# ConwayBeyond/Funscript-Flow

Hardware: AMD Instinct MI355X
Metric: 1080p frame-pairs/sec (higher is better)
Workload: dtype f32

## Files before the change

### funscript_flow_amd/csrc/ffl_api.hip

```cpp
#include "../../include/ffl.h"
#include "ffl_kernels.h"

#include <math.h>
#include <stdarg.h>
#include <stdio.h>
#include <string.h>

#include <algorithm>
#include <condition_variable>
#include <mutex>
#include <string>
#include <thread>
#include <vector>

#define FFL_EV_RING 16
#define FFL_RAW_RING 4

template <class H, class Arg, hipError_t (*Free)(Arg)>
struct Owned {
    H h = H();
    Owned() = default;
    explicit Owned(H take) : h(take) {}
    Owned(Owned &&o) noexcept : h(o.release()) {}
    Owned &operator=(Owned &&o) noexcept { std::swap(h, o.h); return *this; }
// ... 1120 lines not shown
    } pl[3];
    const size_t cw = (size_t)sw / 2 * es, ch = (size_t)sh / 2;
    const size_t wrow = (size_t)yw.w * es, x0 = (size_t)yw.x0 * es;
    pl[0] = {(size_t)yw.y0 * stride_bytes + x0, 0, stride_bytes, wrow, yw.h};
    int np = 3;
    if (nv12) {
        pl[1] = {(size_t)(sh + yw.y0 / 2) * stride_bytes + x0, ybytes, stride_bytes, wrow, yw.h / 2};
        np = 2;
    } else {
        const size_t u0 = (size_t)sh * sw * es + (size_t)(yw.y0 / 2) * cw + x0 / 2;
        pl[1] = {u0, ybytes, (ptrdiff_t)cw, wrow / 2, yw.h / 2};
        pl[2] = {u0 + ch * cw, ybytes + ybytes / 4, (ptrdiff_t)cw, wrow / 2, yw.h / 2};
    }
    const size_t span = (size_t)stride_bytes * (sh + sh / 2 - 1) + (size_t)sw * es;
    auto direct = [&](int i) {
        bool ok = in_host_buf(c, frames[i], span);
        for (int k = 0; ok && k < np; k++) ok = ((uintptr_t)(frames[i] + pl[k].src) | (size_t)pl[k].pitch | pl[k].row) % 4 == 0;
        return ok;
    };
    auto stage = [&](int i, uint8_t *h, int threads) {
        const uint8_t *src[2] = {frames[i] + pl[0].src, nullptr};
        c->pool.copy(h, src, 1, pl[0].pitch, pl[0].row, pl[0].rows, threads);
        src[0] = frames[i] + pl[1].src;
        if (!nv12) src[1] = frames[i] + pl[2].src;
        c->pool.copy(h + pl[1].dst, src, nv12 ? 1 : 2, pl[1].pitch, pl[1].row, pl[1].rows, threads);
    };
    auto send_direct = [&](int i, uint8_t *d) -> int {
        for (int k = 0; k < np; k++)
            HIPCHK(c, hipMemcpy2DAsync(d + pl[k].dst, pl[k].row, frames[i] + pl[k].src, (size_t)pl[k].pitch, pl[k].row,
                                       (size_t)pl[k].rows, hipMemcpyHostToDevice, c->s_copy));
        return FFL_OK;
    };
    auto desc = [&](const uint8_t *d) {
        FrameDesc s = {};
        s.p0 = d;
        s.p1 = d + ybytes;
        s.p2 = nv12 ? s.p1 + es : s.p1 + ybytes / 4;
        s.pitch0 = wrow;
        s.pitch1 = s.pitch2 = nv12 ? wrow : wrow / 2;
        s.c_step = (nv12 ? 2 : 1) * es;
        s.wx = yw.x0;
        s.wy = yw.y0;
        return s;
    };
    return upload_staged(c, lk, first, n, fbytes, fp, direct, stage, send_direct, desc);
}

int ffl_upload_frames_yuv(ffl_ctx *c, int first, int n, const uint8_t *const *frames, int sw, int sh, ptrdiff_t stride_bytes,
                          int layout, int rw, int rh, int crop_x, int crop_y) {
    return upload_yuv(c, "ffl_upload_frames_yuv", first, n, frames, sw, sh, stride_bytes, layout, 1, 8, 0, rw, rh, crop_x, crop_y,
                      nullptr);
}

int ffl_upload_frames_yuv_src(ffl_ctx *c, int first, int n, const uint8_t *const *frames, int sw, int sh, ptrdiff_t stride_bytes,
                              int layout, int rw, int rh, int crop_x, int crop_y, const ffl_source_info *si) {
    return upload_yuv(c, "ffl_upload_frames_yuv", first, n, frames, sw, sh, stride_bytes, layout, 1, 8, 0, rw, rh, crop_x, crop_y, si);
}

int ffl_upload_frames_yuv16(ffl_ctx *c, int first, int n, const uint16_t *const *frames, int sw, int sh, ptrdiff_t stride_bytes,
                            int layout, int depth, int msb_aligned, int rw, int rh, int crop_x, int crop_y) {
    return upload_yuv(c, "ffl_upload_frames_yuv16", first, n, (const uint8_t *const *)frames, sw, sh, stride_bytes, layout, 2,
                      depth, msb_aligned != 0, rw, rh, crop_x, crop_y, nullptr);
}

int ffl_upload_frames_yuv16_src(ffl_ctx *c, int first, int n, const uint16_t *const *frames, int sw, int sh, ptrdiff_t stride_bytes,
                                int layout, int depth, int msb_aligned, int rw, int rh, int crop_x, int crop_y,
                                const ffl_source_info *si) {
    return upload_yuv(c, "ffl_upload_frames_yuv16", first, n, (const uint8_t *const *)frames, sw, sh, stride_bytes, layout, 2,
                      depth, msb_aligned != 0, rw, rh, crop_x, crop_y, si);
}

int ffl_upload_frame(ffl_ctx *c, int fslot, const uint8_t *data, int width, int height, int channels,
                     ptrdiff_t stride_bytes) {
    return ffl_upload_frames(c, fslot, 1, &data, width, height, channels, stride_bytes);
}

int ffl_download_frame(ffl_ctx *c, int fslot, uint8_t *dst) {
    if (!c) return FFL_ERR_INVALID;
    CtxLock lk(c->mu);
    if (!dst || fslot < 0 || fslot >= c->n_fslots)
        return set_err(c, FFL_ERR_INVALID, "ffl_download_frame: bad frame slot %d", fslot);
    if (!c->frame_valid[fslot]) return set_err(c, FFL_ERR_STATE, "ffl_download_frame: frame slot %d was never uploaded", fslot);
    HIPCHK(c, hipSetDevice(c->device));
    HIPCHK(c, hipMemcpyAsync(dst, c->d_gray + (size_t)fslot * c->N, c->N, hipMemcpyDeviceToHost, c->s_copy));
    HIPCHK(c, hipStreamSynchronize(c->s_copy));
    return FFL_OK;
}

struct DebugCapture {
    int level, iter;
    float *I0, *I1, *R0, *R1, *M, *flow;
};

static int enqueue_batch(ffl_ctx *c, ffl_ctx::Lane &L, const BatchTab &T, int n, int nU, int pov_mode, const DebugCapture *cap) {
    hipStream_t st = L.st;
    const size_t N = c->N;
    const UTab *ut = &L.d_tab->ut;
    const PairTab *pt = &L.d_tab->pt;
    auto pyr_level = [&](int k, hipStream_t s) { ffl_launch_pyr_level(c->d_gray, N, ut, nU, L.pyr[c->geo.levels - k], s); };
    auto expand_level = [&](int k, hipStream_t s) {
        {
            ProfScope ps(c, FFL_K_PYRAMID, s);
            pyr_level(k, s);
        }
        {
            ProfScope ps(c, FFL_K_POLYEXP, s);
            ffl_launch_polyexp(L.poly[c->geo.levels - k], nU, c->pc, s);
        }
    };
    const int mode = cap ? 0 : c->opt.run_ahead;
    if (mode) {
        for (int k = 0; k < (mode == 2 ? 4 : 1); k++)
            if (!L.st_aux[k]) HIPCHK(c, hipStreamCreateWithFlags(L.st_aux[k].put(), hipStreamNonBlocking));
        HIPCHK(c, hipEventRecord(L.ev_fork, st));
        for (int k = c->geo.levels; k >= 0; k--) {
            hipStream_t sa = L.st_aux[mode == 2 ? k : 0];
            if (mode == 2 || k == c->geo.levels) HIPCHK(c, hipStreamWaitEvent(sa, L.ev_fork, 0));
            expand_level(k, sa);
            HIPCHK(c, hipEventRecord(L.ev_R[k], sa));
        }
        if (mode == 2)
            for (int k = c->geo.levels; k >= 0; k--) HIPCHK(c, hipStreamWaitEvent(st, L.ev_R[k], 0));
    }
    const bool run_ahead = mode == 1;
    bool expanded = mode != 0;
    if (mode == 0 && c->opt.merge_expand) {
        const PyrJob *l0 = &L.pyr[L.n_jobs - 1];
        const bool fuse_l0 = c->opt.fuse_l0_blur && ffl_polyexp_from_gray_ok(*l0);
        const int skip_l0 = fuse_l0 && !cap;
        {
            ProfScope ps(c, FFL_K_PYRAMID, st);
            if (!ffl_launch_pyr_multi(c->d_gray, N, ut, nU, L.pyr, L.n_jobs - skip_l0, c->opt, st))
                for (int k = c->geo.levels; k >= skip_l0; k--) pyr_level(k, st);
        }
        {
            ProfScope ps(c, FFL_K_POLYEXP, st);
            ffl_launch_polyexp_multi(L.poly, L.n_jobs, nU, c->pc, c->d_gray, N, ut, fuse_l0 ? l0 : nullptr, st);
        }
        expanded = true;
    }

    int pw = 0, ph = 0;
    for (int k = c->geo.levels; k >= 0; k--) {
        const LevelGeom &g = c->geo.lv[k];
        const int lw = g.lw, lh = g.lh;
        const size_t plane = (size_t)lw * lh;
        const size_t I_stride = plane, R_stride = 5 * plane, M_stride = 5 * plane;
        float *Rk = L.d_R + c->lay.r_off[k];
        if (pw == 0 && cap)
            for (int i = 0; i < n; i++) HIPCHK(c, hipMemsetAsync(T.pt.flow[k][i], 0, sizeof(float) * 2 * plane, st));
        if (run_ahead) HIPCHK(c, hipStreamWaitEvent(st, L.ev_R[k], 0));
        else if (!expanded) expand_level(k, st);
        int mi = 0;
        const bool fuse_first = c->opt.fuse_first > 0 && !cap && (long)((lw + 63) / 64) * ((lh + 15) / 16) * n >= c->opt.fuse_first;
        if (!fuse_first) {
            ProfScope ps(c, FFL_K_UPDATE_MATRICES, st);
            ffl_launch_update_matrices(Rk, R_stride, plane, pt, k, n, L.d_M[mi], M_stride, lw, lh, pw, ph, pw == 0, cap != nullptr, c->opt, st);
        }
        bool captured = false;
        auto capture = [&]() -> int {
            HIPCHK(c, hipStreamSynchronize(st));
            if (cap->I0) HIPCHK(c, hipMemcpy(cap->I0, L.d_I + c->lay.i_off[k] + (size_t)T.pt.u0[0] * I_stride, sizeof(float) * plane, hipMemcpyDeviceToHost));
            if (cap->I1) HIPCHK(c, hipMemcpy(cap->I1, L.d_I + c->lay.i_off[k] + (size_t)T.pt.u1[0] * I_stride, sizeof(float) * plane, hipMemcpyDeviceToHost));
            if (cap->R0) HIPCHK(c, hipMemcpy(cap->R0, Rk + (size_t)T.pt.u0[0] * R_stride, sizeof(float) * 5 * plane, hipMemcpyDeviceToHost));
            if (cap->R1) HIPCHK(c, hipMemcpy(cap->R1, Rk + (size_t)T.pt.u1[0] * R_stride, sizeof(float) * 5 * plane, hipMemcpyDeviceToHost));
            if (cap->M) HIPCHK(c, hipMemcpy(cap->M, L.d_M[mi], sizeof(float) * 5 * plane, hipMemcpyDeviceToHost));
            if (cap->flow) HIPCHK(c, hipMemcpy(cap->flow, T.pt.flow[k][0], sizeof(float) * 2 * plane, hipMemcpyDeviceToHost));
            captured = true;
            return FFL_OK;
        };
        for (int it = 0; it < 3; it++) {
            if (cap && cap->level == k && cap->iter == it) {
                int rc = capture();
                if (rc) return rc;
            }
            const int update = it < 2;
            {
                ProfScope ps(c, FFL_K_BLUR_SOLVE, st, it > 0 && !cap);
                if (it == 0 && fuse_first)
                    ffl_launch_blur_solve_first(L.d_M[mi ^ 1], M_stride, Rk, R_stride, plane, pt, k, n, lw, lh, pw, ph, c->opt, st);
                else
                    ffl_launch_blur_solve(L.d_M[mi], L.d_M[mi ^ 1], M_stride, Rk, R_stride, plane, pt, k, n, lw, lh,
                                          update, cap != nullptr, c->opt, st);
            }
            if (update) mi ^= 1;
        }
        if (cap && cap->level == k && !captured) {
            int rc = capture();
            if (rc) return rc;
        }
        pw = lw;
        ph = lh;
    }
    {
        ProfScope ps(c, FFL_K_PASS1, st);
        ffl_launch_pass1(pt, n, c->w, c->h, pov_mode, L.d_pkey, L.d_psum, st);
    }
    return FFL_OK;
}

static int batch_graph(ffl_ctx *c, ffl_ctx::Lane &L, const BatchTab &T, int n, int nU, int pov_mode,
                       ffl_ctx::Lane::GraphEntry **ge) {
    *ge = nullptr;
    for (auto &g : L.graphs)
        if (g.n == n && g.nU == nU && g.pov == pov_mode && g.epoch == c->opt_epoch) *ge = &g;
    if (*ge || c->graph_bad_epoch == c->opt_epoch) return FFL_OK;
    hipStream_t st = L.st;
    ffl_ctx::Lane::GraphEntry g = {n, nU, pov_mode, c->opt_epoch, Graph(), GraphExec()};
    hipError_t fail = hipStreamBeginCapture(st, hipStreamCaptureModeThreadLocal);
    if (fail == hipSuccess) {
        const int rc = enqueue_batch(c, L, T, n, nU, pov_mode, nullptr);
        fail = hipStreamEndCapture(st, g.graph.put());
        if (fail == hipSuccess && (rc != FFL_OK || !g.graph)) fail = hipErrorStreamCaptureInvalidated;
        if (fail == hipSuccess) fail = hipGraphInstantiate(g.exec.put(), g.graph, nullptr, nullptr, 0);
    }
    if (fail != hipSuccess) {
        g.exec.reset();
        g.graph.reset();
        (void)hipGetLastError();
        c->graph_bad_epoch = c->opt_epoch;
        c->graph_failed++;
        if (!c->graph_fail_reported) {
            c->graph_fail_reported = true;
            fprintf(stderr, "libffl_hip: hipGraph capture of a %d-pair batch failed (%s); this context launches its batches "
                            "one kernel at a time until its options change (results are unaffected)\n", n, hipGetErrorString(fail));
        }
        return FFL_OK;
    }
    if (L.graphs.size() >= 16) {
        HIPCHK(c, hipStreamSynchronize(st));
        L.graphs.erase(L.graphs.begin());
    }
    L.graphs.push_back(std::move(g));
    *ge = &L.graphs.back();
    c->graph_captured++;
    return FFL_OK;
}

static int fbg_work(ffl_ctx *c, ffl_ctx::Lane &L, const FbgPlan &p, int nU, FbgWork *wk);

static int queue_batch(ffl_ctx *c, ffl_ctx::Lane &L, BatchTab &T, int *nU_out, int n, const int *f0, const int *f1,
                       const int *slots, int pov_mode, const DebugCapture *cap, const DisKParams *dis,
                       const FbgPlan *fbg) {
    hipStream_t st = L.st;
    const size_t N = c->N;
    int nU = 0;
    auto uidx = [&](int fs) {
        int &u = c->u_of_fslot[fs];
        if (u < 0) {
            T.ut.fslot[nU] = fs;
            u = nU++;
        }
        return u;
    };
    for (int i = 0; i < n; i++) {
        T.pt.u0[i] = uidx(f0[i]);
        T.pt.u1[i] = uidx(f1[i]);
        T.pt.res[i] = c->d_res + slots[i];
    }
    for (int k = c->geo.levels; k >= 0; k--) {
        const size_t plane = (size_t)c->geo.lv[k].lw * c->geo.lv[k].lh;
        float *buf = ((c->geo.levels - k) & 1) ? L.d_flowB : L.d_flowA;
        for (int i = 0; i < n; i++)
            T.pt.flow[k][i] = (k == 0) ? c->d_flow + (size_t)slots[i] * 2 * N : buf + (size_t)i * 2 * plane;
    }
    for (int k = c->geo.levels + 1; k < FFL_MAX_LEVELS; k++)
        for (int i = 0; i < n; i++) T.pt.flow[k][i] = nullptr;
    for (int i = 0; i < nU; i++) c->u_of_fslot[T.ut.fslot[i]] = -1;
    *nU_out = nU;
    WaitOnce wait(st);
    for (int i = 0; i < nU; i++) HIPCHK(c, wait(c->ev_uploaded[T.ut.fslot[i]].get()));
    for (int i = 0; i < n; i++) HIPCHK(c, wait(c->ev_slot_done[slots[i]].get()));
    HIPCHK(c, hipMemcpyAsync(L.d_tab, &T, sizeof(BatchTab), hipMemcpyHostToDevice, st));

    if (fbg || dis) {
        if (fbg) {
            FbgWork wk;
            if (int rc = fbg_work(c, L, *fbg, nU, &wk)) return rc;
            ffl_launch_fb_general(&L.d_tab->ut, &L.d_tab->pt, n, nU, c->d_gray, N, c->w, c->h, *fbg, wk, st);
        } else {
            ffl_launch_dis(&L.d_tab->ut, &L.d_tab->pt, n, c->d_gray, N, L.d_M[0], *dis, st);
        }
        ProfScope ps(c, FFL_K_PASS1, st);
        ffl_launch_pass1(&L.d_tab->pt, n, c->w, c->h, pov_mode, L.d_pkey, L.d_psum, st);
    } else if (c->opt.use_graph && !cap && c->prof_mask == 0 && c->opt.run_ahead == 0) {
        ffl_ctx::Lane::GraphEntry *ge;
        if (int rc = batch_graph(c, L, T, n, nU, pov_mode, &ge)) return rc;
        if (ge) {
            HIPCHK(c, hipGraphLaunch(ge->exec, st));
            c->graph_replayed++;
        } else if (int rc = enqueue_batch(c, L, T, n, nU, pov_mode, nullptr)) {
            return rc;
        }
    } else if (int rc = enqueue_batch(c, L, T, n, nU, pov_mode, cap)) {
        return rc;
    }
    HIPCHK(c, hipGetLastError());
    return FFL_OK;
}

static int run_batch(ffl_ctx *c, int li, int n, const int *f0, const int *f1, const int *slots, int pov_mode,
                     const DebugCapture *cap, const DisKParams *dis = nullptr, const FbgPlan *fbg = nullptr) {
    ffl_ctx::Lane &L = c->lanes[li];
    HIPCHK(c, L.ring.settle_next());
    BatchTab &T = L.h_tab[L.ring.next % FFL_EV_RING];
    int nU = 0;
// ... 959 lines not shown
```

### funscript_flow_amd/csrc/ffl_kernels.h

```cpp
#pragma once
#include <hip/hip_runtime.h>
#include <limits.h>
#include <stdint.h>

#define FFL_MAXB 256
#define FFL_MAXU (2 * FFL_MAXB)
#define FFL_MAX_LEVELS 4
#define FFL_POLY_N 5
#define FFL_WIN 15
#define FFL_WIN_R 7

struct PolyConsts {
    float g[FFL_POLY_N + 1], xg[FFL_POLY_N + 1], xxg[FFL_POLY_N + 1];
    double gd[FFL_POLY_N + 1], xxgd[FFL_POLY_N + 1];
    double ig11, ig03, ig33, ig55;
};

struct GaussKernel {
    float k[32];
    int ksize;
};

struct UTab {
    int fslot[FFL_MAXU];
};

struct PairTab {
    int u0[FFL_MAXB], u1[FFL_MAXB];
    float *flow[FFL_MAX_LEVELS][FFL_MAXB];
    struct Pass1Result *res[FFL_MAXB];
};

struct BatchTab {
    UTab ut;
    PairTab pt;
};

struct Pass1Result {
    int x, y;
    float div_val;
    float pad;
    double mag_sum;
};

enum { FFL_FRONT_GENERIC = 0, FFL_FRONT_AREA2 = 1, FFL_FRONT_IDENTITY = 2 };
enum { FFL_SRC_GRAY = 0, FFL_SRC_BGR = 1, FFL_SRC_YUV = 2, FFL_SRC_YUV16 = 3, FFL_SRC_ANY = -1 };
struct FrameDesc {
    const uint8_t *p0, *p1, *p2;
    long long pitch0, pitch1, pitch2;
    long long ps, cs;
    int c_step;
    int wx, wy;
    int fslot;
};
struct FrontParams {
    int kind, rgb;
    int sw, sh;
    int cx, cy, ow, oh;
    double scale_x, scale_y;
    int mode;
    int shift16, round16;
    int src;
    int ax, bx, cx0, ay, by, cy0;
    int full;
};
struct ExportTab {
    int slot[FFL_MAXB];
};

enum { FFL_IMP_F32 = 0, FFL_IMP_F16 = 1, FFL_IMP_BF16 = 2 };
enum { FFL_IMP_ANY = 0,
       FFL_IMP_NHWC = 1,
       FFL_IMP_NCHW = 2 };
struct ImportArgs {
    const char *base;
    long long item, pitch, ps, cs;
    float *flow;
    Pass1Result *res;
};

#define FFL_MAX_JOBS 4
enum { FFL_PYR_NONE = -1, FFL_PYR_F1 = 0, FFL_PYR_F2, FFL_PYR_H4, FFL_PYR_H9, FFL_PYR_V4, FFL_PYR_V9, FFL_PYR_H1 };
struct PyrJob {
    int kind, w, h, lw, lh;
    unsigned gx, gy, first, count;
    double sx, sy;
    float *tmp, *I;
    size_t tmp_stride, I_stride;
    GaussKernel gk;
};
struct PyrJobs {
    PyrJob j[FFL_MAX_JOBS];
    int n;
};
struct PolyJob {
    const float *I;
    float *R;
    size_t I_stride, R_stride, plane;
    int w, h;
    unsigned gx, gy, first, count;
    int from_gray;
    float gk0, gk1;
};
struct PolyJobs {
    PolyJob j[FFL_MAX_JOBS];
    int n;
};

struct FflOptions {
    int lanes = 2;
    int run_ahead = 0;
    int fuse_first = 10000;
    int merge_expand = 1;
    int use_graph = 1;
    int copy_threads = 4;
    int blur_rows = 0;
    int blur_min_wgs = 3500;
    int tile_order = 0;
    int pyr_coarse = 1;
    int fuse_l0_blur = 1;
    int fb_general = 0;
    int import_fused = 1;
};
struct FflOptionRow {
    const char *name;
    int FflOptions::*member;
    int lo, hi;
    bool flag;
};
inline constexpr FflOptionRow kFflOptionRows[] = {
    {"lanes", &FflOptions::lanes, 1, 4, false},
    {"run_ahead", &FflOptions::run_ahead, 0, 2, false},
    {"fuse_first", &FflOptions::fuse_first, 0, INT_MAX, false},
    {"merge_expand", &FflOptions::merge_expand, INT_MIN, INT_MAX, true},
    {"graph", &FflOptions::use_graph, INT_MIN, INT_MAX, true},
    {"copy_threads", &FflOptions::copy_threads, 1, 16, false},
    {"blur_rows", &FflOptions::blur_rows, 0, 64, false},
    {"blur_min_wgs", &FflOptions::blur_min_wgs, 1, INT_MAX, false},
    {"tile_order", &FflOptions::tile_order, 0, 1, false},
    {"pyr_coarse", &FflOptions::pyr_coarse, INT_MIN, INT_MAX, true},
    {"fuse_l0_blur", &FflOptions::fuse_l0_blur, INT_MIN, INT_MAX, true},
    {"fb_general", &FflOptions::fb_general, 0, 1, false},
    {"import_fused", &FflOptions::import_fused, 0, 1, false},
};

bool ffl_launch_pyr_multi(const uint8_t *gray_base, size_t gray_stride, const UTab *ut, int nU, const PyrJob *levels, int n,
                          const FflOptions &opt, hipStream_t st);
bool ffl_polyexp_from_gray_ok(const PyrJob &l0);
void ffl_launch_polyexp_multi(const PolyJob *levels, int n, int nU, PolyConsts pc, const uint8_t *gray_base, size_t gray_stride,
                              const UTab *ut, const PyrJob *l0, hipStream_t st);
void ffl_launch_frontend(const FrameDesc &d, uint8_t *gray, const FrontParams &p, hipStream_t st);
void ffl_launch_frontend_dev(const FrameDesc *tab, int n, uint8_t *gray_base, size_t N, const FrontParams &p, hipStream_t st);
void ffl_launch_export_flows(const float *flow, const ExportTab &tab, int n, size_t N, char *dst, long long item_stride,
                             int layout, hipStream_t st);
void ffl_launch_import_pass1(const ImportArgs &a, const ExportTab &tab, int n, int dtype, int mode, int w, int h, int pov_mode,
                             int fused, PairTab *pt, unsigned long long *pkey, double *psum, hipStream_t st);
void ffl_launch_gray(const uint8_t *bgr, uint8_t *gray, int n_pixels, hipStream_t st);
size_t ffl_pyr_tmp_floats(int w, int h, int lw);
bool ffl_pyr_level_ok(int w, int h, int lw, int lh, int ksize);
void ffl_launch_pyr_level(const uint8_t *gray_base, size_t gray_stride, const UTab *ut, int nU, const PyrJob &level,
                          hipStream_t st);
void ffl_launch_polyexp(const PolyJob &level, int nU, PolyConsts pc, hipStream_t st);
void ffl_launch_update_matrices(const float *R, size_t R_stride, size_t plane, const PairTab *pt, int level, int nB, float *M,
                                size_t M_stride, int lw, int lh, int pw, int ph, int zero_flow, int store_flow,
                                const FflOptions &opt, hipStream_t st);
void ffl_launch_blur_solve(const float *Min, float *Mout, size_t M_stride, const float *R, size_t R_stride,
                           size_t plane, const PairTab *pt, int level, int nB, int lw, int lh, int update, int store_flow,
                           const FflOptions &opt, hipStream_t st);


void ffl_launch_blur_solve_first(float *Mout, size_t M_stride, const float *R, size_t R_stride, size_t plane,
                                 const PairTab *pt, int level, int nB, int lw, int lh, int pw, int ph, const FflOptions &opt,
                                 hipStream_t st);

#define DIS_MAX_PATCHES 4096
#define DIS_MAX_SCALES 12
struct DisKParams {
    int w, h, finest, coarsest, stride, gd_iters, vr_iters, mean_norm, spatial_prop, stripes;
    float alpha, gamma, delta;
    size_t pair_floats;
    size_t pyr_floats;
    size_t pyr_off[DIS_MAX_SCALES];
    float *dbg;
    int dbg_scale, dbg_stage;
};
void ffl_launch_dis(const UTab *ut, const PairTab *pt, int nB, const uint8_t *gray, size_t gray_stride, float *scratch,
                    const DisKParams &p, hipStream_t st);

int ffl_pass1_blocks(int w, int h);
void ffl_launch_pass1(const PairTab *pt, int nB, int w, int h, int pov_mode, unsigned long long *pkey, double *psum,
                      hipStream_t st);

#define FFL_WINDOW_MAX_RADIUS 32
struct WindowSeq {
    int slot[FFL_MAXB + 2 * FFL_WINDOW_MAX_RADIUS];
};
struct WindowItem {
    const float *flow;
    double cx, cy;
    int cut, pad;
};
struct Pass2Record {
    double dot, cx, cy;
    float mean_mag, div_val;
    int x, y, cut, pad;
};
void ffl_launch_radial(const WindowItem *tab, int n, int w, int h, int pov_mode, const double *wytab, double *psum,
                       Pass2Record *out, hipStream_t st);
void ffl_launch_window_plan(const WindowSeq &seq, int n_seq, int first, int n, int radius, float cut_threshold,
                            const Pass1Result *res, const float *flow, int w, int h, WindowItem *tab, Pass2Record *out,
                            hipStream_t st);

__device__ __forceinline__ int ffl_clampi(int v, int lo, int hi) { return v < lo ? lo : (v > hi ? hi : v); }

__device__ __forceinline__ int ffl_reflect101(int p, int n) {
    if (n == 1) return 0;
    while (p < 0 || p >= n) p = p < 0 ? -p : 2 * (n - 1) - p;
    return p;
}

__device__ __forceinline__ void ffl_resize_coord(int d, int src, double scale, int &i0, int &i1, float &f) {
    float fx = (float)((d + 0.5) * scale - 0.5);
    int sx = (int)floorf(fx);
    fx -= sx;
    if (sx < 0) { sx = 0; fx = 0.f; }
    if (sx >= src - 1) { sx = src - 1; fx = 0.f; }
    i0 = sx;
    i1 = sx + 1 < src ? sx + 1 : src - 1;
    f = fx;
}

static inline unsigned ffl_xcd_blocks(unsigned count) { return ((count + 7) / 8) * 8; }
__device__ __forceinline__ bool ffl_xcd_tile(unsigned l, unsigned count, unsigned &t) {
    const unsigned chunk = (count + 7) >> 3;
    t = (l & 7u) * chunk + (l >> 3);
    return (l >> 3) < chunk && t < count;
}

#ifndef FFL_PANEL_W
#define FFL_PANEL_W 4
#endif
static inline unsigned ffl_tile_grid(int tiles_x, int tiles_y, int nB) {
    const int T = tiles_x * tiles_y;
    return (unsigned)(((T + 7) / 8) * 8 * nB);
}
__device__ __forceinline__ bool ffl_tile_coord(int tiles_x, int tiles_y, int nB, int order, int &b, int &tile_x,
                                               int &tile_y) {
    const int T = tiles_x * tiles_y, chunk = (T + 7) >> 3;
    int t;
    if (order == 0) {
        b = blockIdx.x / (chunk * 8);
        const int l = blockIdx.x - b * (chunk * 8);
        t = (l & 7) * chunk + (l >> 3);
    } else {
        const int pos = blockIdx.x >> 3, tt = pos / nB;
        b = pos - tt * nB;
        t = (blockIdx.x & 7) * chunk + tt;
    }
    if (t >= T) return false;
    const int per_panel = FFL_PANEL_W * tiles_y;
    const int panel = t / per_panel, within = t - panel * per_panel;
    const int pw = min(FFL_PANEL_W, tiles_x - panel * FFL_PANEL_W);
    tile_y = within / pw;
    tile_x = panel * FFL_PANEL_W + (within - tile_y * pw);
    return true;
}

#define FFL_GLOBAL __attribute__((address_space(1)))
typedef float ffl_v2f __attribute__((ext_vector_type(2), aligned(4)));
typedef float ffl_v4f __attribute__((ext_vector_type(4), aligned(4)));
__device__ __forceinline__ float2 ffl_gload2(const void *base, size_t byte_off) {
    const ffl_v2f v = *(const FFL_GLOBAL ffl_v2f *)((const char *)base + byte_off);
    return make_float2(v.x, v.y);
}
__device__ __forceinline__ float4 ffl_gload4(const void *base, size_t byte_off) {
    const ffl_v4f v = *(const FFL_GLOBAL ffl_v4f *)((const char *)base + byte_off);
    return make_float4(v.x, v.y, v.z, v.w);
}

struct __attribute__((packed, aligned(4))) ffl_f2u { float x, y; };
struct __attribute__((packed, aligned(4))) ffl_f4u { float x, y, z, w; };

template <typename T>
__device__ __forceinline__ const T *ffl_at(const float *base, unsigned idx) {
    return reinterpret_cast<const T *>(reinterpret_cast<const char *>(base) + idx * 4u);
}
template <typename T>
__device__ __forceinline__ T *ffl_at(float *base, unsigned idx) {
    return reinterpret_cast<T *>(reinterpret_cast<char *>(base) + idx * 4u);
}

__device__ __forceinline__ ffl_f2u ffl_ld_corner(const float *plane_base, unsigned idx) {
    ffl_f2u v;
    v.x = *ffl_at<float>(plane_base, idx);
    v.y = *ffl_at<float>(plane_base, idx + 1u);
    return v;
}

struct UmLoc {
    int x1, y1;
    float a00, a01, a10, a11;
    bool inside;
};
__device__ __forceinline__ UmLoc ffl_um_locate(int w, int h, int x, int y, float dx, float dy) {
    UmLoc L;
    float fx = x + dx, fy = y + dy;
    L.x1 = (int)floorf(fx);
    L.y1 = (int)floorf(fy);
    fx -= L.x1;
    fy -= L.y1;
    L.inside = (unsigned)L.x1 < (unsigned)(w - 1) && (unsigned)L.y1 < (unsigned)(h - 1);
    L.a00 = (1.f - fx) * (1.f - fy);
    L.a01 = fx * (1.f - fy);
    L.a10 = (1.f - fx) * fy;
    L.a11 = fx * fy;
    return L;
}

__device__ __forceinline__ void ffl_um_finish(const float (&r0)[5], const float (&b)[5], bool inside, int w, int h, int x,
                                              int y, float dx, float dy, float (&out)[5]) {
#define FFL_BORDER(i) ((i) < 2 ? 0.14f : 0.4472f)
    float r2 = inside ? b[0] : 0.f;
    float r3 = inside ? b[1] : 0.f;
    float r4 = inside ? (r0[2] + b[2]) * 0.5f : r0[2];
    float r5 = inside ? (r0[3] + b[3]) * 0.5f : r0[3];
    float r6 = inside ? (r0[4] + b[4]) * 0.25f : r0[4] * 0.5f;
    r2 = (r0[0] - r2) * 0.5f;
// ... 53 lines not shown
```

### funscript_flow_amd/csrc/kernels_farneback.hip

```cpp
#include "ffl_kernels.h"

__global__ __launch_bounds__(256) void k_gray(const uint8_t *__restrict__ bgr, uint8_t *__restrict__ gray, int n) {
    int i4 = (blockIdx.x * 256 + threadIdx.x) * 4;
    if (i4 + 3 < n) {
        const uint32_t *p = reinterpret_cast<const uint32_t *>(bgr + (size_t)i4 * 3);
        uint32_t a = p[0], b = p[1], c = p[2];
        uint32_t px[12] = {a & 255, (a >> 8) & 255, (a >> 16) & 255, a >> 24, b & 255, (b >> 8) & 255,
                           (b >> 16) & 255, b >> 24, c & 255, (c >> 8) & 255, (c >> 16) & 255, c >> 24};
        uint32_t o = 0;
#pragma unroll
        for (int j = 0; j < 4; j++) {
            uint32_t g = (px[j * 3] * 3735u + px[j * 3 + 1] * 19235u + px[j * 3 + 2] * 9798u + 16384u) >> 15;
            o |= g << (8 * j);
        }
        *reinterpret_cast<uint32_t *>(gray + i4) = o;
    } else {
        for (int i = i4; i < n; i++) {
            uint32_t b = bgr[(size_t)i * 3], g = bgr[(size_t)i * 3 + 1], r = bgr[(size_t)i * 3 + 2];
            gray[i] = (uint8_t)((b * 3735u + g * 19235u + r * 9798u + 16384u) >> 15);
        }
    }
}

void ffl_launch_gray(const uint8_t *bgr, uint8_t *gray, int n_pixels, hipStream_t st) {
// ... 1094 lines not shown
                const unsigned lane_byte = ((unsigned)((c0 + vcc) * plane) + (unsigned)vgx) * 4u;
                if (FIRST) {
#pragma unroll
                    for (int j = 0; j < NCARRY; j++) v[j] = carry[g][j];
#pragma unroll
                    for (int j = 0; j < TH; j++)
                        v[NCARRY + j] = g == 0 ? sM012[(vcc * TH + j) * UP + vtx] : sM34[c0 - GC + vcc][j][vtx];
                } else {
                    if (rb == 0) {
#pragma unroll
                        for (int j = 0; j < NCARRY; j++) {
                            const unsigned gy = (unsigned)min(max(y0 + j - FFL_WIN_R, 0), h - 1);
                            v[j] = *reinterpret_cast<const float *>(Mbb + (gy * pitch + lane_byte));
                        }
                    } else {
#pragma unroll
                        for (int j = 0; j < NCARRY; j++) v[j] = carry[g][j];
                    }
#pragma unroll
                    for (int j = NCARRY; j < LH; j++) {
                        const unsigned gy = (unsigned)min(max(y0 + j - FFL_WIN_R, 0), h - 1);
                        v[j] = *reinterpret_cast<const float *>(Mbb + (gy * pitch + lane_byte));
                    }
                }
            }
            if (FIRST && g == 0) __syncthreads();
            if (vlane) {
#pragma unroll
                for (int j = 0; j < NCARRY; j++) carry[g][j] = v[TH + j];
                double o[TH];
                ffl_box_block16(v, o);
                const int pos = vtx + 2 * (vtx >> 4);
#pragma unroll
                for (int j = 0; j < TH; j++) sS[(vcc * TH + j) * (2 * LW2) + pos] = o[j];
            }
            FFL_T(4)
            __syncthreads();
            FFL_T(5)
#pragma unroll
            for (int cc = 0; cc < GC; cc++) {
                if (cc >= nc) break;
                double d[PX + 14];
                const double2 *src = &sS2[cc][ty][9 * kk];
#define FFL_K5_H(Q)                                                                        \
    {                                                                                      \
        _Pragma("unroll") for (int j = 0; j < (PX + 14) / 2; j++) {                        \
            const double2 t2 = src[2 * (Q) + j + ((4 * (Q) + 2 * j) >> 4)];                \
            d[2 * j] = t2.x;                                                               \
            d[2 * j + 1] = t2.y;                                                           \
        }                                                                                  \
        ffl_box_quarter<Q>(d, acc[c0 + cc]);                                               \
    }
                switch (q) {
                    case 0: FFL_K5_H(0) break;
                    case 1: FFL_K5_H(1) break;
                    case 2: FFL_K5_H(2) break;
                    default: FFL_K5_H(3) break;
                }
#undef FFL_K5_H
            }
        }

        FFL_T(6)
        __syncthreads();
        FFL_T(7)
        {
            float2 f[PX];
#pragma unroll
            for (int p = 0; p < PX; p++) {
                double g11 = acc[0][p] * scale, g12 = acc[1][p] * scale, g22 = acc[2][p] * scale,
                       h1 = acc[3][p] * scale, h2 = acc[4][p] * scale;
                double idet = 1.0 / (g11 * g22 - g12 * g12 + 1e-3);
                f[p].x = (float)((g11 * h2 - g12 * h1) * idet);
                f[p].y = (float)((g22 * h1 - g12 * h2) * idet);
            }
            sF4[(ty * FP + lx0) / 2] = make_float4(f[0].x, f[0].y, f[1].x, f[1].y);
            sF4[(ty * FP + lx0) / 2 + 1] = make_float4(f[2].x, f[2].y, f[3].x, f[3].y);
        }
        FFL_T(8)
        __syncthreads();
        FFL_T(9)
        if (UPDATE) {
            const int lx = tid & 63, x = min(x0 + lx, w - 1);
            const float2 *sF2 = reinterpret_cast<const float2 *>(sF4);
            ffl_um_rows<TH / 4>(R0, R1, Mo, plane, w, h, x, x0 + lx < w, y0 + (tid >> 6),
                                [&](int k) { return sF2[((tid >> 6) + 4 * k) * FP + lx]; },
                                [&](unsigned o, float2 d) {
                                    if (store_flow) *reinterpret_cast<float2 *>(ffl_at<float>(reinterpret_cast<float *>(flow), 2u * o)) = d;
                                });
        } else {
            const int lx = 2 * (tid & 31), x = x0 + lx;
            if (x < w) {
                const bool second = x + 1 < w;
#pragma unroll
                for (int k = 0; k < TH / 8; k++) {
                    const int ly = (tid >> 5) + 8 * k;
                    if (y0 + ly >= h) continue;
                    const float4 ff = sF4[(ly * FP + lx) >> 1];
                    const size_t o = (size_t)(y0 + ly) * w + x;
                    if (second) {
                        ffl_f4u t;
                        t.x = ff.x; t.y = ff.y; t.z = ff.z; t.w = ff.w;
                        *reinterpret_cast<ffl_f4u *>(flow + o) = t;
                    } else {
                        flow[o] = make_float2(ff.x, ff.y);
                    }
                }
            }
        }
        FFL_T(10)
        __syncthreads();
        FFL_T(11)
    }
#ifdef FFL_STAMP
    if (FFL_STAMP_ON && tid == 0)
        for (int i = 0; i < FFL_NSTAMP; i++) g_stamp[blockIdx.x & 63][i] = sStamp[i];
#endif
}

static int ffl_blur_rows_per_wg(int tiles_x, int tiles_y, int nB, int min_wgs) {
    if (nB > 32 && tiles_x * tiles_y >= 256) nB = 32;
    for (int s = 1; s <= tiles_y; s++) {
        const int nrb = (tiles_y + s - 1) / s;
        if (nrb > 64) continue;
        if ((long)tiles_x * ((tiles_y + nrb - 1) / nrb) * nB >= min_wgs || nrb == 1) return nrb;
    }
    return 1;
}

template <typename K>
static void ffl_launch_k5(K k, const float *Min, float *Mout, size_t M_stride, const float *R, size_t R_stride, size_t plane,
                          const PairTab *pt, int level, int nB, int lw, int lh, int pw, int ph, int store_flow,
                          const FflOptions &opt, hipStream_t st) {
    const int tiles_x = (lw + 63) / 64, tiles_y = (lh + 15) / 16;
    const int nrb = opt.blur_rows > 0 ? opt.blur_rows : ffl_blur_rows_per_wg(tiles_x, tiles_y, nB, opt.blur_min_wgs);
    dim3 grid(ffl_tile_grid(tiles_x, (tiles_y + nrb - 1) / nrb, nB));
    hipLaunchKernelGGL(k, grid, dim3(256), 0, st, Min, Mout, M_stride, R, R_stride, plane, pt, level, lw, lh, nrb, pw, ph,
                       pw > 0 ? (double)pw / lw : 1.0, pw > 0 ? (double)ph / lh : 1.0, store_flow, nB, opt.tile_order);
}

void ffl_launch_blur_solve(const float *Min, float *Mout, size_t M_stride, const float *R, size_t R_stride,
                           size_t plane, const PairTab *pt, int level, int nB, int lw, int lh, int update, int store_flow,
                           const FflOptions &opt, hipStream_t st) {
    ffl_launch_k5(update ? k_blur_solve<true, 0> : k_blur_solve<false, 0>, Min, Mout, M_stride, R, R_stride, plane, pt, level,
                  nB, lw, lh, 0, 0, update ? store_flow : 1, opt, st);
}

void ffl_launch_blur_solve_first(float *Mout, size_t M_stride, const float *R, size_t R_stride, size_t plane,
                                 const PairTab *pt, int level, int nB, int lw, int lh, int pw, int ph, const FflOptions &opt,
                                 hipStream_t st) {
    ffl_launch_k5(pw > 0 ? k_blur_solve<true, 1> : k_blur_solve<true, 2>, (const float *)nullptr, Mout, M_stride, R, R_stride,
                  plane, pt, level, nB, lw, lh, pw, ph, 0, opt, st);
}
```

Baseline: 6431.

## Solve coarsest Farneback level in one LDS-resident kernel per pair

When the coarsest pyramid level is small enough (up to about 32x32) to fit in LDS, all three update/blur/solve iterations now run in a single workgroup per pair. The matrices, column sums and displacement stay in shared memory, with barriers between the stages. This replaces several small kernel launches with one and avoids round trips through global memory for the intermediates. The trade-off is low parallelism: only one workgroup per pair, using close to 64KB of LDS. The change also adds a host-side index checker for the LDS layout.

```diff
diff --git a/funscript_flow_amd/csrc/check/level_lds_index_check.cpp b/funscript_flow_amd/csrc/check/level_lds_index_check.cpp
--- /dev/null
+++ b/funscript_flow_amd/csrc/check/level_lds_index_check.cpp
@@ -0,0 +1,128 @@
+#include <cstdio>
+#include <cstdlib>
+#include <vector>
+
+#include "../ffl_level_lds.h"
+
+static long g_checks = 0;
+#define REQUIRE(cond, ...)                                  \
+    do {                                                    \
+        g_checks++;                                         \
+        if (!(cond)) {                                      \
+            std::fprintf(stderr, "FAILED %s: ", #cond);     \
+            std::fprintf(stderr, __VA_ARGS__);              \
+            std::fprintf(stderr, "\n");                     \
+            std::exit(1);                                   \
+        }                                                   \
+    } while (0)
+
+struct Region {
+    int *g;
+    int n;
+    const char *name;
+    Region(int n_, const char *nm) : g(static_cast<int *>(std::calloc(n_ > 0 ? n_ : 1, sizeof(int)))), n(n_), name(nm) {}
+    ~Region() { std::free(g); }
+    void write(int i, int gen, int w, int h) {
+        REQUIRE(i >= 0 && i < n, "%s write %d of %d at %dx%d", name, i, n, w, h);
+        g[i] = gen;
+    }
+    void read(int i, int gen, int w, int h) {
+        REQUIRE(i >= 0 && i < n, "%s read %d of %d at %dx%d", name, i, n, w, h);
+        REQUIRE(g[i] == gen, "%s element %d read in generation %d holds %d at %dx%d", name, i, gen, g[i], w, h);
+    }
+};
+
+static void walk(int w, int h) {
+    const LvlLayout L = ffl_lvl_layout(w, h);
+    REQUIRE(L.bytes <= FFL_LVL_LDS_BYTES && L.s_off % 16 == 0 && L.s_off >= 4 * L.m_floats && L.bytes == L.s_off + 8 * L.s_doubles,
+            "layout of %dx%d: %d bytes", w, h, L.bytes);
+    REQUIRE(8 * L.f_float2s <= 8 * L.s_doubles, "displacement of %dx%d outgrows the column sums it aliases", w, h);
+    REQUIRE(h * L.nbx <= 64, "%dx%d: %d quads per quarter", w, h, h * L.nbx);
+    Region M(L.m_floats, "sM"), S(L.s_doubles, "sS"), F(L.f_float2s, "sF"), G(w * h, "flow");
+    const int npix = w * h, ppass = ffl_lvl_passes(npix), vitems = ffl_lvl_v_items(L), vpass = ffl_lvl_passes(vitems);
+    int gen = 1;
+    for (int p = 0; p < ppass; p++)
+        for (int tid = 0; tid < FFL_LVL_THREADS; tid++) {
+            const int i = ffl_lvl_pixel(L, p, tid), y = i / w;
+            F.write(ffl_lvl_f_index(L, i - y * w, y), gen, w, h);
+        }
+    for (int y = 0; y < h; y++)
+        for (int x = 0; x < w; x++) F.read(ffl_lvl_f_index(L, x, y), gen, w, h);
+    for (int it = 0; it < 3; it++) {
+        for (int tid = 0; tid < FFL_LVL_THREADS; tid++) {
+            for (int p = 0; p <= ppass; p++) {
+                const int pass = p < ppass - 1 ? p : ppass - 1;
+                const int i = ffl_lvl_pixel(L, pass, tid), y = i / w, x = i - y * w;
+                REQUIRE(i >= 0 && i < npix && x >= 0 && x < w && y >= 0 && y < h, "pixel %d at %dx%d", i, w, h);
+                F.read(ffl_lvl_f_index(L, x, y), gen, w, h);
+            }
+            for (int p = 0; p < ppass; p++) {
+                if (p * FFL_LVL_THREADS + tid >= npix) continue;
+                const int i = ffl_lvl_pixel(L, p, tid), y = i / w, x = i - y * w;
+                REQUIRE(i == p * FFL_LVL_THREADS + tid, "unclamped pixel");
+                for (int c = 0; c < 5; c++) {
+                    REQUIRE(M.g[ffl_lvl_m_index(L, c, x, y)] != gen + 1, "M written twice at %dx%d", w, h);
+                    M.write(ffl_lvl_m_index(L, c, x, y), gen + 1, w, h);
+                }
+            }
+        }
+        gen++;
+        for (int i = 0; i < L.m_floats; i++) M.read(i, gen, w, h);
+        for (int i = 0; i < L.f_float2s; i++) F.g[i] = -1;
+        for (int p = 0; p < vpass; p++)
+            for (int tid = 0; tid < FFL_LVL_THREADS; tid++) {
+                const int i = p * FFL_LVL_THREADS + tid;
+                if (i >= vitems) continue;
+                const LvlVItem V = ffl_lvl_v_item(L, i);
+                REQUIRE(V.c >= 0 && V.c < 5 && V.kb >= 0 && V.kb < L.nby && V.x >= 0 && V.x < w, "V item %d at %dx%d", i, w, h);
+                for (int j = 0; j < 30; j++) M.read(ffl_lvl_v_read(L, V, j), gen, w, h);
+                for (int t = 0; t < 16; t++) {
+                    REQUIRE(S.g[ffl_lvl_v_write(L, V, t)] != gen, "column sum written twice at %dx%d", w, h);
+                    S.write(ffl_lvl_v_write(L, V, t), gen, w, h);
+                }
+            }
+        for (int tid = 0; tid < FFL_LVL_THREADS; tid++) {
+            const int q = tid >> 6;
+            const LvlHItem H = ffl_lvl_h_item(L, tid & 63);
+            REQUIRE(H.r >= 0 && H.r < h && H.kk >= 0 && H.kk < L.nbx, "H item of lane %d at %dx%d", tid, w, h);
+            for (int c = 0; c < 5; c++)
+                for (int j = 0; j < 18; j++) S.read(ffl_lvl_h_read(L, H, c, q, j), gen, w, h);
+        }
+        for (int i = 0; i < L.s_doubles; i++) S.g[i] = -1;
+        for (int tid = 0; tid < FFL_LVL_THREADS; tid++) {
+            const int q = tid >> 6;
+            const LvlHItem H = ffl_lvl_h_item(L, tid & 63);
+            for (int p = 0; p < 4; p++) {
+                const int o = ffl_lvl_h_write(L, H, q, p);
+                if (o < 0) continue;
+                REQUIRE(F.g[o] != gen, "displacement written twice at %dx%d", w, h);
+                F.write(o, gen, w, h);
+            }
+        }
+        for (int y = 0; y < h; y++)
+            for (int x = 0; x < w; x++) F.read(ffl_lvl_f_index(L, x, y), gen, w, h);
+    }
+    for (int p = 0; p < ppass; p++)
+        for (int tid = 0; tid < FFL_LVL_THREADS; tid++) {
+            const int i = p * FFL_LVL_THREADS + tid, ic = ffl_lvl_pixel(L, p, tid), y = ic / w;
+            F.read(ffl_lvl_f_index(L, ic - y * w, y), gen, w, h);
+            if (i < npix) G.write(i, gen, w, h);
+        }
+    for (int i = 0; i < npix; i++) G.read(i, gen, w, h);
+}
+
+int main() {
+    static_assert(ffl_lvl_fits(32, 32) && ffl_lvl_layout(32, 32).bytes == 62720, "the reference's operating point");
+    int sizes = 0, largest = 0;
+    for (int h = 0; h <= FFL_LVL_MAX_SIDE + 1; h++)
+        for (int w = 0; w <= FFL_LVL_MAX_SIDE + 1; w++) {
+            if (!ffl_lvl_fits(w, h)) continue;
+            walk(w, h);
+            sizes++;
+            if (ffl_lvl_layout(w, h).bytes > largest) largest = ffl_lvl_layout(w, h).bytes;
+        }
+    REQUIRE(ffl_lvl_fits(32, 32) && ffl_lvl_fits(31, 25) && ffl_lvl_fits(33, 17) && !ffl_lvl_fits(64, 32) && !ffl_lvl_fits(65, 33) &&
+            !ffl_lvl_fits(33, 33) && !ffl_lvl_fits(1, 8), "the rule's landmarks");
+    std::printf("level_lds_index_check: %d eligible sizes, largest workgroup %d bytes, %ld checks ok\n", sizes, largest, g_checks);
+    return 0;
+}
diff --git a/funscript_flow_amd/csrc/ffl_api.hip b/funscript_flow_amd/csrc/ffl_api.hip
--- a/funscript_flow_amd/csrc/ffl_api.hip
+++ b/funscript_flow_amd/csrc/ffl_api.hip
@@ -1296,6 +1296,15 @@
         if (run_ahead) HIPCHK(c, hipStreamWaitEvent(st, L.ev_R[k], 0));
         else if (!expanded) expand_level(k, st);
         int mi = 0;
+        if (c->opt.coarse_one_launch && !cap && ffl_level_one_launch_ok(lw, lh, pw)) {
+            {
+                ProfScope ps(c, FFL_K_BLUR_SOLVE, st);
+                ffl_launch_level_lds(Rk, R_stride, plane, pt, k, n, lw, lh, st);
+            }
+            pw = lw;
+            ph = lh;
+            continue;
+        }
         const bool fuse_first = c->opt.fuse_first > 0 && !cap && (long)((lw + 63) / 64) * ((lh + 15) / 16) * n >= c->opt.fuse_first;
         if (!fuse_first) {
             ProfScope ps(c, FFL_K_UPDATE_MATRICES, st);
diff --git a/funscript_flow_amd/csrc/ffl_kernels.h b/funscript_flow_amd/csrc/ffl_kernels.h
--- a/funscript_flow_amd/csrc/ffl_kernels.h
+++ b/funscript_flow_amd/csrc/ffl_kernels.h
@@ -2,6 +2,8 @@
 #include <hip/hip_runtime.h>
 #include <limits.h>
 #include <stdint.h>
+
+#include "ffl_level_lds.h"
 
 #define FFL_MAXB 256
 #define FFL_MAXU (2 * FFL_MAXB)
@@ -121,6 +123,7 @@
     int fuse_l0_blur = 1;
     int fb_general = 0;
     int import_fused = 1;
+    int coarse_one_launch = 1;
 };
 struct FflOptionRow {
     const char *name;
@@ -142,6 +145,7 @@
     {"fuse_l0_blur", &FflOptions::fuse_l0_blur, INT_MIN, INT_MAX, true},
     {"fb_general", &FflOptions::fb_general, 0, 1, false},
     {"import_fused", &FflOptions::import_fused, 0, 1, false},
+    {"coarse_one_launch", &FflOptions::coarse_one_launch, INT_MIN, INT_MAX, true},
 };
 
 bool ffl_launch_pyr_multi(const uint8_t *gray_base, size_t gray_stride, const UTab *ut, int nU, const PyrJob *levels, int n,
@@ -173,6 +177,10 @@
                                  const PairTab *pt, int level, int nB, int lw, int lh, int pw, int ph, const FflOptions &opt,
                                  hipStream_t st);
 
+bool ffl_level_one_launch_ok(int lw, int lh, int pw);
+void ffl_launch_level_lds(const float *R, size_t R_stride, size_t plane, const PairTab *pt, int level, int nB, int lw, int lh,
+                          hipStream_t st);
+
 #define DIS_MAX_PATCHES 4096
 #define DIS_MAX_SCALES 12
 struct DisKParams {
diff --git a/funscript_flow_amd/csrc/ffl_level_lds.h b/funscript_flow_amd/csrc/ffl_level_lds.h
--- /dev/null
+++ b/funscript_flow_amd/csrc/ffl_level_lds.h
@@ -0,0 +1,88 @@
+#pragma once
+
+#ifdef __HIPCC__
+#define FFL_LVL_HD __host__ __device__ __forceinline__ constexpr
+#else
+#define FFL_LVL_HD inline constexpr
+#endif
+
+#define FFL_LVL_THREADS 256
+#define FFL_LVL_LDS_BYTES 65536
+#define FFL_LVL_MAX_SIDE 64
+
+struct LvlLayout {
+    int w, h;
+    int nbx, nby;
+    int sp, fp;
+    int m_floats, s_doubles, f_float2s;
+    int s_off;
+    int bytes;
+};
+
+FFL_LVL_HD int ffl_lvl_clamp(int v, int lo, int hi) { return v < lo ? lo : (v > hi ? hi : v); }
+
+FFL_LVL_HD LvlLayout ffl_lvl_layout(int w, int h) {
+    LvlLayout L = {};
+    L.w = w;
+    L.h = h;
+    L.nbx = (w + 15) / 16;
+    L.nby = (h + 15) / 16;
+    L.sp = w | 1;
+    L.fp = w | 1;
+    L.m_floats = 5 * w * h;
+    L.s_doubles = 5 * 16 * L.nby * L.sp;
+    L.f_float2s = h * L.fp;
+    L.s_off = (4 * L.m_floats + 15) / 16 * 16;
+    L.bytes = L.s_off + 8 * L.s_doubles;
+    return L;
+}
+
+FFL_LVL_HD bool ffl_lvl_fits(int w, int h) {
+    if (w < 2 || h < 2 || w > FFL_LVL_MAX_SIDE || h > FFL_LVL_MAX_SIDE) return false;
+    const LvlLayout L = ffl_lvl_layout(w, h);
+    return h * L.nbx <= 64 && L.f_float2s <= L.s_doubles && L.bytes <= FFL_LVL_LDS_BYTES;
+}
+
+FFL_LVL_HD int ffl_lvl_passes(int n_items) { return (n_items + FFL_LVL_THREADS - 1) / FFL_LVL_THREADS; }
+FFL_LVL_HD int ffl_lvl_pixel(const LvlLayout &L, int pass, int tid) {
+    return ffl_lvl_clamp(pass * FFL_LVL_THREADS + tid, 0, L.w * L.h - 1);
+}
+FFL_LVL_HD int ffl_lvl_f_index(const LvlLayout &L, int x, int y) { return y * L.fp + x; }
+FFL_LVL_HD int ffl_lvl_m_index(const LvlLayout &L, int c, int x, int y) { return (c * L.h + y) * L.w + x; }
+
+struct LvlVItem {
+    int c, kb, x;
+};
+FFL_LVL_HD int ffl_lvl_v_items(const LvlLayout &L) { return 5 * L.nby * L.w; }
+FFL_LVL_HD LvlVItem ffl_lvl_v_item(const LvlLayout &L, int i) {
+    LvlVItem V = {};
+    V.c = i / (L.nby * L.w);
+    const int rem = i - V.c * (L.nby * L.w);
+    V.kb = rem / L.w;
+    V.x = rem - V.kb * L.w;
+    return V;
+}
+FFL_LVL_HD int ffl_lvl_v_read(const LvlLayout &L, const LvlVItem &V, int j) {
+    return ffl_lvl_m_index(L, V.c, V.x, ffl_lvl_clamp(16 * V.kb - 7 + j, 0, L.h - 1));
+}
+FFL_LVL_HD int ffl_lvl_s_index(const LvlLayout &L, int c, int x, int row) { return (c * 16 * L.nby + row) * L.sp + x; }
+FFL_LVL_HD int ffl_lvl_v_write(const LvlLayout &L, const LvlVItem &V, int t) { return ffl_lvl_s_index(L, V.c, V.x, 16 * V.kb + t); }
+
+struct LvlHItem {
+    bool on;
+    int r, kk;
+};
+FFL_LVL_HD LvlHItem ffl_lvl_h_item(const LvlLayout &L, int lane) {
+    LvlHItem H = {};
+    H.on = lane < L.h * L.nbx;
+    H.kk = H.on ? lane / L.h : 0;
+    H.r = H.on ? lane - H.kk * L.h : 0;
+    return H;
+}
+FFL_LVL_HD int ffl_lvl_h_read(const LvlLayout &L, const LvlHItem &H, int c, int q, int j) {
+    return ffl_lvl_s_index(L, c, ffl_lvl_clamp(16 * H.kk + 4 * q - 7 + j, 0, L.w - 1), H.r);
+}
+FFL_LVL_HD int ffl_lvl_h_write(const LvlLayout &L, const LvlHItem &H, int q, int p) {
+    const int x = 16 * H.kk + 4 * q + p;
+    return H.on && x < L.w ? ffl_lvl_f_index(L, x, H.r) : -1;
+}
diff --git a/funscript_flow_amd/csrc/kernels_farneback.hip b/funscript_flow_amd/csrc/kernels_farneback.hip
--- a/funscript_flow_amd/csrc/kernels_farneback.hip
+++ b/funscript_flow_amd/csrc/kernels_farneback.hip
@@ -1270,3 +1270,135 @@
     ffl_launch_k5(pw > 0 ? k_blur_solve<true, 1> : k_blur_solve<true, 2>, (const float *)nullptr, Mout, M_stride, R, R_stride,
                   plane, pt, level, nB, lw, lh, pw, ph, 0, opt, st);
 }
+
+static_assert(ffl_lvl_fits(32, 32) && ffl_lvl_layout(32, 32).bytes == 62720,
+              "a 32 x 32 level: 20480 B of M + 42240 B of column sums (the displacement aliases them)");
+static_assert(!ffl_lvl_fits(64, 32), "a 64 x 32 level would need 124160 B: one workgroup per CU, not taken");
+
+__global__ __launch_bounds__(FFL_LVL_THREADS) void k_level_lds(const float *__restrict__ R, size_t R_stride, size_t plane,
+                                                               const PairTab *__restrict__ pt, int level, int w, int h) {
+    extern __shared__ double2 ffl_lvl_smem[];
+    const LvlLayout L = ffl_lvl_layout(w, h);
+    float *sM = reinterpret_cast<float *>(ffl_lvl_smem);
+    double *sS = reinterpret_cast<double *>(reinterpret_cast<char *>(ffl_lvl_smem) + L.s_off);
+    float2 *sF = reinterpret_cast<float2 *>(sS);
+    const int tid = threadIdx.x, b = blockIdx.x;
+    const float *R0 = R + (size_t)pt->u0[b] * R_stride, *R1 = R + (size_t)pt->u1[b] * R_stride;
+    float2 *flow = reinterpret_cast<float2 *>(pt->flow[level][b]);
+    const int npix = w * h, ppass = ffl_lvl_passes(npix), vpass = ffl_lvl_passes(ffl_lvl_v_items(L));
+    const double scale = 1.0 / (FFL_WIN * FFL_WIN);
+    const int q = __builtin_amdgcn_readfirstlane(tid >> 6);
+    const LvlHItem H = ffl_lvl_h_item(L, tid & 63);
+
+    for (int p = 0; p < ppass; p++) {
+        const int i = ffl_lvl_pixel(L, p, tid), y = i / w;
+        sF[ffl_lvl_f_index(L, i - y * w, y)] = make_float2(0.f, 0.f);
+    }
+    __syncthreads();
+
+#pragma unroll 1
+    for (int it = 0; it < 3; it++) {
+        {
+            struct UmPix {
+                int x, y;
+                float2 f;
+                float a00, a01, a10, a11;
+                bool inside;
+                float r0[5];
+                ffl_f2u t[5], u[5];
+            };
+            auto issue = [&](int pass) {
+                UmPix S;
+                const int i = ffl_lvl_pixel(L, pass, tid);
+                S.y = i / w;
+                S.x = i - S.y * w;
+                S.f = sF[ffl_lvl_f_index(L, S.x, S.y)];
+#pragma unroll
+                for (int c = 0; c < 5; c++) S.r0[c] = *ffl_at<float>(R0 + c * plane, (unsigned)i);
+                const UmLoc U = ffl_um_locate(w, h, S.x, S.y, S.f.x, S.f.y);
+                S.a00 = U.a00; S.a01 = U.a01; S.a10 = U.a10; S.a11 = U.a11; S.inside = U.inside;
+                const unsigned o1 = U.inside ? (unsigned)U.y1 * (unsigned)w + (unsigned)U.x1 : 0u;
+#pragma unroll
+                for (int c = 0; c < 5; c++) {
+                    S.t[c] = ffl_ld_corner(R1 + c * plane, o1);
+                    S.u[c] = ffl_ld_corner(R1 + c * plane, o1 + (unsigned)w);
+                }
+                return S;
+            };
+            UmPix cur = issue(0);
+#pragma unroll 1
+            for (int p = 0; p < ppass; p++) {
+                const UmPix nxt = issue(min(p + 1, ppass - 1));
+                float bb[5];
+#pragma unroll
+                for (int c = 0; c < 5; c++) bb[c] = cur.a00 * cur.t[c].x + cur.a01 * cur.t[c].y + cur.a10 * cur.u[c].x + cur.a11 * cur.u[c].y;
+                float m[5];
+                ffl_um_finish(cur.r0, bb, cur.inside, w, h, cur.x, cur.y, cur.f.x, cur.f.y, m);
+                if (p * FFL_LVL_THREADS + tid < npix) {
+#pragma unroll
+                    for (int c = 0; c < 5; c++) sM[ffl_lvl_m_index(L, c, cur.x, cur.y)] = m[c];
+                }
+                cur = nxt;
+            }
+        }
+        __syncthreads();
+#pragma unroll 1
+        for (int p = 0; p < vpass; p++) {
+            const int i = p * FFL_LVL_THREADS + tid;
+            if (i < ffl_lvl_v_items(L)) {
+                const LvlVItem V = ffl_lvl_v_item(L, i);
+                float v[30];
+#pragma unroll
+                for (int j = 0; j < 30; j++) v[j] = sM[ffl_lvl_v_read(L, V, j)];
+                double o[16];
+                ffl_box_block16(v, o);
+#pragma unroll
+                for (int t = 0; t < 16; t++) sS[ffl_lvl_v_write(L, V, t)] = o[t];
+            }
+        }
+        __syncthreads();
+        double acc[5][4];
+#pragma unroll
+        for (int c = 0; c < 5; c++) {
+            double d[18];
+#define FFL_LVL_H(Q)                                                                      \
+    {                                                                                     \
+        _Pragma("unroll") for (int j = 0; j < 18; j++) d[j] = sS[ffl_lvl_h_read(L, H, c, Q, j)]; \
+        ffl_box_quarter<Q>(d, acc[c]);                                                    \
+    }
+            switch (q) {
+                case 0: FFL_LVL_H(0) break;
+                case 1: FFL_LVL_H(1) break;
+                case 2: FFL_LVL_H(2) break;
+                default: FFL_LVL_H(3) break;
+            }
+#undef FFL_LVL_H
+        }
+        __syncthreads();
+#pragma unroll
+        for (int p = 0; p < 4; p++) {
+            double g11 = acc[0][p] * scale, g12 = acc[1][p] * scale, g22 = acc[2][p] * scale,
+                   h1 = acc[3][p] * scale, h2 = acc[4][p] * scale;
+            double idet = 1.0 / (g11 * g22 - g12 * g12 + 1e-3);
+            float2 f;
+            f.x = (float)((g11 * h2 - g12 * h1) * idet);
+            f.y = (float)((g22 * h1 - g12 * h2) * idet);
+            const int o = ffl_lvl_h_write(L, H, q, p);
+            if (o >= 0) sF[o] = f;
+        }
+        __syncthreads();
+    }
+    for (int p = 0; p < ppass; p++) {
+        const int i = p * FFL_LVL_THREADS + tid, ic = ffl_lvl_pixel(L, p, tid), y = ic / w;
+        const float2 f = sF[ffl_lvl_f_index(L, ic - y * w, y)];
+        if (i < npix) flow[i] = f;
+    }
+}
+
+bool ffl_level_one_launch_ok(int lw, int lh, int pw) { return pw == 0 && ffl_lvl_fits(lw, lh); }
+
+void ffl_launch_level_lds(const float *R, size_t R_stride, size_t plane, const PairTab *pt, int level, int nB, int lw, int lh,
+                          hipStream_t st) {
+    hipLaunchKernelGGL(k_level_lds, dim3(nB), dim3(FFL_LVL_THREADS), (size_t)ffl_lvl_layout(lw, lh).bytes, st, R, R_stride, plane,
+                       pt, level, lw, lh);
+}
```

Result: no change. 6448, median of 2 (+0.3%).
